# kangxiongbin/HyLight

Measured on AMD Instinct MI355X. Metric: long-read all-vs-all overlaps/sec, higher is better.
Workload: dtype u8/int32

## Files before the change

hylight_amd/csrc/ava_align.hip:

```cpp
#include <algorithm>
#include <memory>
#include <type_traits>

#include "ava_internal.h"
#include "dev_prims.h"
#include "wave_ops.h"

namespace hlmi {

namespace {
constexpr int WG = 256;
constexpr int WAVES = WG / 64;
constexpr int SEQ_T_MAX = EXT_MAX + BAND_W;
constexpr int NR_SHORT = 128;
constexpr int WIDE_SHORT = 128;
inline dim3 grid1(size_t n) { return grid_for(n, WG); }

struct Task {
    uint32_t piece;
    uint16_t kind;
    uint16_t narrow;
    uint64_t qa, ta;
    int16_t m, n;
    int16_t dlo;
    int16_t trim;
};
constexpr uint16_t TASK_REV = 4;
constexpr uint16_t TASK_ONE = 8;
struct TaskOut {
    int32_t score;
    int32_t bi, bj;
    uint32_t runs_off, n_runs;
    uint32_t pad;
};
__device__ __forceinline__ uint32_t end_codes(uint32_t first_run, uint32_t last_run) { return (first_run & 15u) | (last_run & 15u) << 4; }

__global__ void piece_task_count_kernel(const Piece *pieces, size_t n, uint32_t *cnt) {
    size_t i = blockIdx.x * (size_t)blockDim.x + threadIdx.x;
    if (i < n) cnt[i] = pieces[i].n_fp + 1;
}

struct TaskRef { uint32_t pk, fp; };
struct PieceGeom {
    uint64_t qo, to;
    uint32_t ql, tl;
    uint32_t strand;
    uint32_t stub_cand;
};
struct TaskGeom {
    const TaskRef *ref;
    const PieceGeom *pg;
    const FixPt *fps;
};
__device__ __forceinline__ Task build_task(const PieceGeom &p, uint32_t piece, uint32_t kind, FixPt f0, FixPt f1, int ext_max) {
    const int ql = (int)p.ql, tl = (int)p.tl;
    const uint64_t qo = p.qo, to = p.to;
    const uint16_t rev = p.strand ? TASK_REV : 0;
    auto qaddr = [&](int pos) { return p.strand ? qo + (uint64_t)(ql - 1 - pos) : qo + (uint64_t)pos; };
    if (kind == 1) {
        const int qs = (int)f0.q, ts = (int)f0.t;
        const int m = qs < ext_max ? qs : ext_max, n2 = ts < m + BAND_W ? ts : m + BAND_W;
        return Task{piece, (uint16_t)(1u | rev), (uint16_t)(qs <= ext_max ? (qs + 1) << 1 : 0), qaddr(qs - 1),
                    to + (uint64_t)(ts - 1), (int16_t)m, (int16_t)n2, (int16_t)(-(BAND_W / 2 - 1)), 0};
    }
    if (kind == 2) {
        const int qe = (int)f0.q, te = (int)f0.t;
        const int m = ql - qe < ext_max ? ql - qe : ext_max, n2 = tl - te < m + BAND_W ? tl - te : m + BAND_W;
        return Task{piece, (uint16_t)(2u | rev), (uint16_t)(ql - qe <= ext_max ? (ql - qe + 1) << 1 : 0), qaddr(qe),
// ... 51 lines not shown
    if (stub_oh >= 0) {
        const FixPt a = fps[p.fp_off], b = fps[p.fp_off + p.n_fp - 1];
        const uint32_t dq = (uint32_t)(ext_max + stub_oh), dt = (uint32_t)(ext_max + BAND_W + stub_oh);
        cand = ((a.q > dq && a.t > dt) || (ql - b.q > dq && tl - b.t > dt)) ? 1u : 0u;
    }
    pg[i] = PieceGeom{qoff[p.q], toff[p.t], ql, tl, p.strand, cand};
}

struct AlignArgs {
    Task *tasks;
    TaskGeom geom;
    size_t n_tasks;
    const uint32_t *list;
    size_t n_list;
    const uint8_t *qcodes, *tcodes;
    long long q_total, t_total;
    const uint8_t *qpacked, *tpacked;
    const uint32_t *qnflag, *tnflag;
    int match, mismatch, go, ge, ambi;
    int go2, ge2;
    int end_bonus;
    int ext_max;
    int ext_all_long;
    int ungapped;
    int kmax;
    int kgap1;
    int kgap2;
    int one_ok;
    int kext_plain;
    int kext_bonus;
    int trim_ok;
    int kshift;
    TaskOut *out;
    uint32_t *runs;
    uint32_t cap_runs;
    uint32_t *counters;
    uint32_t run_buf_cap;
    uint8_t *cls_bare;
    uint8_t *defer_flag;
    const uint32_t *defer_list, *defer_count;
};

__device__ __forceinline__ uint32_t wave_excl_sum_u32(uint32_t v, int lane, uint32_t &total) {
    (void)lane;
    const uint32_t x = wave_prefix_sum_incl_dpp(v);
    total = (uint32_t)__builtin_amdgcn_readlane((int)x, 63);
    return x - v;
}

constexpr uint32_t RUN_CHUNK = 4096;
constexpr uint32_t RUN_CHUNK_SMALL = 256;
__device__ __forceinline__ uint32_t pool_take(const AlignArgs &a, uint32_t n, uint32_t &chunk_off, uint32_t &chunk_left,
                                              bool &ok, uint32_t chunk = RUN_CHUNK) {
    if (n > chunk_left) {
        const uint32_t want = n > chunk ? n : chunk;
        chunk_off = atomicAdd(&a.counters[0], want);
        chunk_left = want;
        if ((unsigned long long)chunk_off + want > a.cap_runs) { a.counters[1] = 1; chunk_left = 0; ok = false; return 0; }
    }
    const uint32_t off = chunk_off;
    chunk_off += n;
    chunk_left -= n;
    return off;
}

__device__ __forceinline__ uint32_t load_codes4(const uint8_t *base, long long idx, long long total) {
    if (idx >= 0 && idx + 4 <= total) {
        uint32_t v;
        __builtin_memcpy(&v, base + idx, 4);
        return v;
    }
    uint32_t v = 0;
    for (int k = 0; k < 4; ++k) v |= (uint32_t)(idx + k >= 0 && idx + k < total ? base[idx + k] : 4) << (8 * k);
    return v;
}
__device__ __forceinline__ uint32_t comp_codes4(uint32_t x) {
    const uint32_t n = x & 0x04040404u;
    return (x ^ 0x03030303u) & ~((n >> 1) | (n >> 2));
}
__device__ __forceinline__ uint32_t load_window4(const uint8_t *codes, long long total, long long a0, bool down, bool comp, int x) {
    uint32_t v = down ? __builtin_bswap32(load_codes4(codes, a0 - x - 3, total)) : load_codes4(codes, a0 + x, total);
    if (comp) v = comp_codes4(v);
    return v;
}

__device__ __forceinline__ uint32_t load_window4p(const uint8_t *codes, long long a0, bool down, bool comp, int x) {
    uint32_t v;
    __builtin_memcpy(&v, codes + (down ? a0 - x - 3 : a0 + x), 4);
    if (down) v = __builtin_bswap32(v);
    if (comp) v = comp_codes4(v);
    return v;
}


enum { ST_BASES = 0, ST_BASES_SQUARE, ST_BASES_NARROW, ST_BASES_WIDE, ST_FAST, ST_DP, ST_DP_ROWS, ST_NARROW_SMALL, ST_WIDE_ONE, ST_STUB_EXT, ST_EXT_CERT, ST_EXT_DP_ROW, ST_EXT_DP_K, ST_LONG, ST_BASES_LONG, ST_PACKED, N_ALIGN_STATS };
constexpr int NR_SMALL = 64;
constexpr uint8_t CLS_LONG = 5;
constexpr uint8_t CLS_LONG32 = 7;
constexpr uint8_t CLS_UNGAPPED = 6;

__device__ __forceinline__ uint64_t load_codes8(const uint8_t *base, long long idx, long long total) {
    if (idx >= 0 && idx + 8 <= total) {
        uint64_t v;
        __builtin_memcpy(&v, base + idx, 8);
        return v;
    }
    uint64_t v = 0;
    for (int k = 0; k < 8; ++k) v |= (uint64_t)(idx + k >= 0 && idx + k < total ? base[idx + k] : 4) << (8 * k);
    return v;
}
__device__ __forceinline__ uint64_t load_window8(const uint8_t *codes, long long total, long long a0, bool down, bool comp, int x) {
    uint64_t v = down ? __builtin_bswap64(load_codes8(codes, a0 - x - 7, total)) : load_codes8(codes, a0 + x, total);
    if (comp) {
        const uint64_t n = v & 0x0404040404040404ull;
        v = (v ^ 0x0303030303030303ull) & ~((n >> 1) | (n >> 2));
    }
    return v;
}

__device__ __forceinline__ uint64_t load_window8p(const uint8_t *codes, long long a0, bool down, bool comp, int x) {
    uint64_t v;
    __builtin_memcpy(&v, codes + (down ? a0 - x - 7 : a0 + x), 8);
    if (down) v = __builtin_bswap64(v);
    if (comp) {
        const uint64_t n = v & 0x0404040404040404ull;
        v = (v ^ 0x0303030303030303ull) & ~((n >> 1) | (n >> 2));
    }
    return v;
// ... 37 lines not shown
    for (uint32_t w = g0 >> 5; w <= g1 >> 5; ++w) {
        uint32_t keep = ~0u;
        if (w == g0 >> 5) keep &= ~0u << (g0 & 31);
        if (w == g1 >> 5) keep &= ~0u >> (31 - (g1 & 31));
        any |= nflag[w] & keep;
    }
    return any != 0;
}
__device__ __forceinline__ bool window_flagged(const uint32_t *nflag, long long a0, bool down, int len) {
    return down ? range_flagged(nflag, a0 - (len - 1), a0) : range_flagged(nflag, a0, a0 + (len - 1));
}

template <int PASS>
__global__ __launch_bounds__(WG) __attribute__((amdgpu_waves_per_eu(PASS == 1 ? 4 : 5))) void classify_kernel(AlignArgs a, uint8_t *cls, unsigned long long *stats) {
    __shared__ unsigned long long s_stat[WAVES][N_ALIGN_STATS];
    constexpr int CMP_WORDS = PASS == 1 ? 64 * (BLOCK_MAX / 32) : 1;
    __shared__ uint32_t s_mm[WAVES][CMP_WORDS], s_up[WAVES][CMP_WORDS], s_dn[WAVES][CMP_WORDS];
    __shared__ uint64_t s_qa[WAVES][PASS == 1 ? 64 : 1], s_ta[WAVES][PASS == 1 ? 64 : 1];
    __shared__ uint32_t s_geo[WAVES][PASS == 1 ? 64 : 1], s_amb[WAVES][2];
    const int lane = threadIdx.x & 63;
    const size_t tid = blockIdx.x * (size_t)blockDim.x + threadIdx.x;
    const size_t n_thr = (size_t)gridDim.x * blockDim.x;
    uint32_t chunk_off = 0, chunk_left = 0;
    uint32_t st[N_ALIGN_STATS] = {};
    const size_t n_units = PASS == 1 ? a.n_tasks : (size_t)*a.defer_count;
    const size_t rounds = (n_units + n_thr - 1) / n_thr;
    TaskRef ref_n{0, 0};
    uint32_t ti_n = 0;
    if (PASS == 1) { if (tid < n_units) ref_n = a.geom.ref[tid]; }
    else if (tid < n_units) ti_n = a.defer_list[tid];
    for (size_t r = 0; r < rounds; ++r) {
        const size_t u = r * n_thr + tid;
        bool live = u < n_units;
        const size_t ti = PASS == 1 || !live ? u : (size_t)ti_n;
        TaskRef ref = ref_n;
        if (PASS == 2 && live) ref = a.geom.ref[ti];
        {
            const size_t un = u + n_thr;
            if (PASS == 1) { if (un < n_units) ref_n = a.geom.ref[un]; }
            else if (un < n_units) ti_n = a.defer_list[un];
        }
        Task tk{};
        bool held = false;
        bool bare = false;
        if (live) {
            const uint32_t pc = ref.pk & 0x3fffffffu, kind = ref.pk >> 30;
            const PieceGeom pg = a.geom.pg[pc];
            held = PASS == 1 && kind != 0 && pg.stub_cand != 0;
            bare = a.cls_bare != nullptr && pg.stub_cand != 0;
            const FixPt f0 = a.geom.fps[ref.fp];
            FixPt f1{0, 0};
            if (kind == 0) f1 = a.geom.fps[ref.fp + 1];
            tk = build_task(pg, pc, kind, f0, f1, a.ext_max);
        }
        const int m = tk.m, n = tk.n;
        uint8_t c = 2;
        bool try_fast = false;
        if (live) {
            if (m <= 0 || n <= 0 || held) c = 0;
            else if ((tk.kind & 3) == 0) {
                if (m > BLOCK_MAX || n > BLOCK_MAX)
                    c = (n > m ? n - m : m - n) <= HALF_DELTA ? CLS_LONG32 : CLS_LONG;
                else { c = tk.narrow ? (m <= NR_SHORT ? 1 : 3) : 2; try_fast = (m == n); }
            } else if ((m < n - tk.dlo ? m : n - tk.dlo) > EXT_MAX) { c = CLS_LONG32; tk.dlo = (int16_t)(-(HALF_W / 2 - 1)); }
            else if (a.ext_all_long) c = CLS_LONG;
            if (c == 2 && (m < n - tk.dlo ? m : n - tk.dlo) <= WIDE_SHORT) c = 4;
// ... 318 lines not shown
                        const int xp = k ? xpos2 : xpos;
                        if (xp < from || xp >= to) continue;
                        if (xp > prev) runs[nr++] = (uint32_t)(xp - prev) << 4 | OP_EQ;
                        if (nr && xp == prev && prev > from && (runs[nr - 1] & 15u) == OP_X) runs[nr - 1] += 1u << 4;
                        else runs[nr++] = 1u << 4 | OP_X;
                        prev = xp + 1;
                    }
                    if (to > prev) runs[nr++] = (uint32_t)(to - prev) << 4 | OP_EQ;
                };
                seg(0, p_star);
                runs[nr++] = (uint32_t)gap << 4 | (del ? OP_D : OP_I);
                seg(p_star, mn);
                const int subs = (xpos >= 0 ? 1 : 0) + (xpos2 >= 0 ? 1 : 0);
                int gap_cost = a.go + a.ge * gap;
                if (a.go2 && a.go2 + a.ge2 * gap < gap_cost) gap_cost = a.go2 + a.ge2 * gap;
                fast_score = a.match * (mn - subs) - a.mismatch * subs - gap_cost;
                fast = true;
                c = 0;
            }
        } else if (fast) {
            c = 0;
            int prev = 0, xs = -1, xe = -1;
            for (int i = 0; i < k; ++i) {
                const int x = mpos[i];
                if (x == xe) { xe = x + 1; continue; }
                if (xs >= 0) { runs[nr++] = (uint32_t)(xe - xs) << 4 | OP_X; prev = xe; }
                if (x > prev) runs[nr++] = (uint32_t)(x - prev) << 4 | OP_EQ;
                xs = x; xe = x + 1;
            }
            if (xs >= 0) { runs[nr++] = (uint32_t)(xe - xs) << 4 | OP_X; prev = xe; }
            if (m > prev) runs[nr++] = (uint32_t)(m - prev) << 4 | OP_EQ;
        }
        if (bare) nr = 0;
        uint32_t wave_total;
        const uint32_t mine = wave_excl_sum_u32(nr, lane, wave_total);
        uint32_t base = 0;
        bool ok = true;
        if (wave_total) {
            if (lane == 0) base = pool_take(a, wave_total, chunk_off, chunk_left, ok);
            base = (uint32_t)__shfl((int)base, 0, 64);
            ok = __shfl((int)ok, 0, 64) != 0;
        }
        if (fast) {
            if (ok) for (uint32_t q = 0; q < nr; ++q) a.runs[base + mine + q] = runs[q];
            const bool ext = (tk.kind & 3) != 0;
            const int L = ext_take >= 0 ? ext_take : (m < n ? m : n);
            a.out[ti] = TaskOut{fast_score, ext ? L : m, ext ? L : n, base + mine, ok ? nr : 0, (nr ? end_codes(runs[0], runs[nr - 1]) : 0u) | ext_flag};
        } else if (live && c == 0) {
            a.out[ti] = TaskOut{0, 0, 0, 0, 0, 0};
        }
        int m_dp = m;
        if (live && !fast && (c == 1 || c == 3) && a.kmax >= 0 && last_x >= 0 && a.trim_ok && !a.ungapped) {
            const int mn = m < n ? m : n;
            int T = mn - 1 - last_x;
            T = T < mn - 1 ? T : mn - 1;
            if (T > 0) {
                tk.m = (int16_t)(m - T); tk.n = (int16_t)(n - T); tk.trim = (int16_t)T;
                m_dp = m - T;
                c = m_dp <= NR_SHORT ? 1 : 3;
            }
        }
        if (live) {
            if (a.ungapped && c != 0) c = CLS_UNGAPPED;
            cls[ti] = bare ? 0 : c;
            if (a.cls_bare) a.cls_bare[ti] = bare ? c : 0;
            if (c != 0) a.tasks[ti] = tk;
            if (held) ++st[ST_STUB_EXT];
            else if (m > 0 && n > 0) {
                const uint32_t bases = (uint32_t)(m + n);
                st[ST_BASES] += bases;
                if ((tk.kind & 3) == 0 && m == n) st[ST_BASES_SQUARE] += bases;
                if (c == 0) ++st[ST_FAST];
                else {
                    ++st[ST_DP];
                    if (c == CLS_LONG || c == CLS_LONG32) { ++st[ST_LONG]; st[ST_BASES_LONG] += bases; st[ST_DP_ROWS] += (uint32_t)(m < n - tk.dlo ? m : n - tk.dlo); }
                    else if (c == 2 || c == 4) { st[ST_BASES_WIDE] += bases; st[ST_DP_ROWS] += (uint32_t)(m < n - tk.dlo ? m : n - tk.dlo); }
                    else { st[ST_BASES_NARROW] += bases; st[ST_DP_ROWS] += (uint32_t)m_dp; if (c == 1 && m_dp < NR_SMALL && !bare) ++st[ST_NARROW_SMALL]; }
                }
            }
        }
    }
// ... 1249 lines not shown
            base = (uint32_t)__shfl((int)base, 0, 64);
            ok = __shfl((int)ok, 0, 64) != 0;
        }
        if (live && ok && n_runs) {
            uint32_t k = 0, len = 0;
            int op_cur = -1;
            uint32_t *dst = a.runs + base + mine;
            auto put = [&]() { dst[left ? n_runs - 1 - k : k] = len << 4 | (uint32_t)op_cur; ++k; };
            for (int x = 0; x < take; x += 8) {
                uint64_t q8, t8;
                pair_at(x, q8, t8);
                const int lim = take - x < 8 ? take - x : 8;
                for (int y = 0; y < lim; ++y) {
                    const int op = ((q8 >> (8 * y)) & 0xff) == ((t8 >> (8 * y)) & 0xff) ? (int)OP_EQ : (int)OP_X;
                    if (op != op_cur) { if (len) put(); op_cur = op; len = 0; }
                    ++len;
                }
            }
            if (len) put();
        }
        if (live) {
            const uint32_t ends = n_runs ? (left ? end_codes(last_op, first_op) : end_codes(first_op, last_op)) : 0u;
            a.out[ti] = TaskOut{out_score, ext ? take : (int)tk.m, ext ? take : (int)tk.n, base + mine, ok ? n_runs : 0,
                                ends | (ext && take == end_row ? 0x80000000u : 0u)};
        }
    }
}

struct AsmArgs {
    const Piece *pieces;
    const FixPt *fps;
    const uint32_t *task_off;
    const TaskOut *tout;
    const uint32_t *runs;
    size_t n_pieces;
    const uint32_t *qlen, *tlen, *rank_q, *rank_t, *chunk_of_t;
    int min_dp_score, end_bonus;
    const uint32_t *plist;
    const PieceGeom *pg;
    uint8_t *late;
    int stub_score;
    int bare;
    uint32_t stage_cap;
};

constexpr uint32_t ASM_MID = 4;
constexpr int ASM_STAGE = 1024;
template <bool WRITE>
__global__ __launch_bounds__(WG) void assemble_kernel(AsmArgs a, uint32_t *n_ops, uint8_t *valid, const uint64_t *ops_off,
                                                       uint32_t *ops, PafRec *recs, uint64_t *ord_hi, uint64_t *ord_lo) {
    __shared__ uint32_t s_stage[WRITE ? WAVES : 1][WRITE ? ASM_STAGE : 1];
    uint32_t *const stage = s_stage[WRITE ? (threadIdx.x >> 6) : 0];
    const int lane = threadIdx.x & 63;
    const size_t wave = (blockIdx.x * (size_t)blockDim.x + threadIdx.x) >> 6;
    const size_t n_waves = ((size_t)gridDim.x * blockDim.x) >> 6;
    for (size_t idx = wave; idx < a.n_pieces; idx += n_waves) {
        const size_t i = !WRITE && a.plist ? (size_t)a.plist[idx] : idx;
        if (WRITE && !valid[i]) continue;
        const Piece p = a.pieces[i];
        const FixPt *fp = a.fps + p.fp_off;
        const TaskOut *to = a.tout + a.task_off[i];
        const uint32_t n_tasks = p.n_fp + 1;
        const bool bare = a.bare && a.pg[i].stub_cand != 0;
        uint32_t *w = WRITE ? ops + ops_off[i] : nullptr;
        long long score = 0;
        unsigned long long nmatch = 0, blen = 0;
        uint32_t slots = 0;
        uint32_t carry_code = 99;
        constexpr uint32_t NO_SLOT = 0xffffffffu;
        uint32_t open_idx = NO_SLOT, open_val = 0;
        int ext_l_i = 0, ext_l_j = 0, ext_r_i = 0, ext_r_j = 0;
        TaskOut r_next{0, 0, 0, 0, 0, 0};
        if ((uint32_t)lane < n_tasks) r_next = to[lane];
        for (uint32_t t0 = 0; t0 < n_tasks; t0 += 64) {
            const uint32_t t = t0 + (uint32_t)lane;
            TaskOut r = r_next;
            r_next = TaskOut{0, 0, 0, 0, 0, 0};
            if (t + 64 < n_tasks) r_next = to[t + 64];
            bool keep = false;
            if (t < n_tasks) {
                keep = true;
                if (t == 0 || t == n_tasks - 1)
                    keep = !(r.score + ((r.pad & 0x80000000u) ? a.end_bonus : 0) <= 0 || (r.n_runs == 0 && !bare));
            }
            if (keep && t == 0) { ext_l_i = r.bi; ext_l_j = r.bj; }
            if (keep && t == n_tasks - 1 && t != 0) { ext_r_i = r.bi; ext_r_j = r.bj; }
            long long sc = keep ? r.score : 0;
            const uint32_t nr = keep && !bare ? r.n_runs : 0;
            const uint32_t first = r.pad & 15u, last = (r.pad >> 4) & 15u;
            const unsigned long long ne_mask = __ballot(nr != 0);
            const unsigned long long below = ne_mask & ((1ull << lane) - 1ull);
            const int prev_lane = below ? 63 - __clzll((long long)below) : 0;
            const uint32_t prev_last = (uint32_t)__shfl((int)last, prev_lane, 64);
            const uint32_t prev_code = below ? (prev_last & 15u) : carry_code;
            const bool mrg = nr != 0 && (first & 15u) == prev_code;
            uint32_t tot_runs, tot_mrg;
            const uint32_t S = wave_excl_sum_u32(nr, lane, tot_runs);
            const uint32_t Mx = wave_excl_sum_u32(mrg ? 1u : 0u, lane, tot_mrg);
            if (WRITE) {
                const uint32_t F = nr ? a.runs[r.runs_off] : 0u;
                const uint32_t L = nr >= 2 ? a.runs[r.runs_off + nr - 1] : F;
                uint32_t mid[ASM_MID];
#pragma unroll
                for (uint32_t u = 0; u < ASM_MID; ++u) mid[u] = u + 3 <= nr ? a.runs[r.runs_off + 1 + u] : 0u;
                const uint32_t P = wave_prefix_sum_incl_dpp(mrg ? F >> 4 : 0u);
                const bool opens = nr != 0 && (!mrg || nr >= 2);
                const unsigned long long om = __ballot(opens);
                const uint32_t P_end = (uint32_t)__builtin_amdgcn_readlane((int)P, 63);
                const uint32_t T0 = om ? (uint32_t)__shfl((int)P, __ffsll((long long)om) - 1, 64) : P_end;
                open_val += T0 << 4;
                if (om && open_idx != NO_SLOT && lane == 0) w[open_idx] = open_val;
                const unsigned long long above = lane == 63 ? 0ull : om & ~((2ull << lane) - 1ull);
                const uint32_t P_next = (uint32_t)__shfl((int)P, above ? __ffsll((long long)above) - 1 : 63, 64);
                const uint32_t base = slots + S - (Mx + (mrg ? 1u : 0u));
                const uint32_t own_slot = base + (nr ? nr - 1 : 0u);
                const uint32_t own_val = L + ((P_next - P) << 4);
                const uint32_t n_out = tot_runs - tot_mrg;
                const bool staged = n_out <= a.stage_cap;
                auto put = [&](uint32_t slot, uint32_t v) { if (staged) stage[slot - slots] = v; else w[slot] = v; };
                if (om) {
                    const int lb = 63 - __clzll((long long)om);
                    open_idx = (uint32_t)__builtin_amdgcn_readlane((int)own_slot, lb);
                    open_val = (uint32_t)__builtin_amdgcn_readlane((int)own_val, lb);
                    if (opens && lane != lb) put(own_slot, own_val);
                }
                if (nr) {
                    blen += F >> 4;
                    if ((F & 15u) == OP_EQ) nmatch += F >> 4;
                }
                if (nr >= 2) {
                    blen += L >> 4;
                    if ((L & 15u) == OP_EQ) nmatch += L >> 4;
                    if (!mrg) put(base, F);
// ... 42 lines not shown
        for (int o = 32; o > 0; o >>= 1) { nmatch += __shfl_xor(nmatch, o, 64); blen += __shfl_xor(blen, o, 64); }
        if (lane == 0) {
            if (open_idx != NO_SLOT) w[open_idx] = open_val;
            const int qs = (int)fp[0].q - li, ts = (int)fp[0].t - lj;
            const int qe = (int)fp[p.n_fp - 1].q + ri, te = (int)fp[p.n_fp - 1].t + rj;
            const uint32_t ql = a.qlen[p.q];
            PafRec r{};
            r.qid = a.rank_q[p.q]; r.tid = a.rank_t[p.t];
            r.qlen = ql; r.tlen = a.tlen[p.t];
            r.qs = p.strand ? ql - (uint32_t)qe : (uint32_t)qs;
            r.qe = p.strand ? ql - (uint32_t)qs : (uint32_t)qe;
            r.ts = (uint32_t)ts; r.te = (uint32_t)te;
            r.nmatch = (uint32_t)nmatch; r.blen = (uint32_t)blen;
            r.flags = p.strand ? PF_REV : 0;
            r.chunk = a.chunk_of_t[p.t];
            r.cig_off = ops_off[i]; r.cig_n = slots; r.tie = 0;
            recs[i] = r;
            ord_hi[i] = (uint64_t)r.chunk << 32 | p.q;
            ord_lo[i] = (uint64_t)p.t << 43 | (uint64_t)p.strand << 42 | (uint64_t)(p.chain & 0x3fffffu) << 20 | (p.piece & 0xfffffu);
        }
    }
}

template <bool WRITE>
__global__ __launch_bounds__(WG) void assemble_lane_kernel(AsmArgs a, uint32_t *n_ops, uint8_t *valid, const uint64_t *ops_off,
                                                            uint32_t *ops, PafRec *recs, uint64_t *ord_hi, uint64_t *ord_lo) {
    const size_t idx = blockIdx.x * (size_t)blockDim.x + threadIdx.x;
    if (idx >= a.n_pieces) return;
    const size_t i = !WRITE && a.plist ? (size_t)a.plist[idx] : idx;
    if (WRITE && !valid[i]) return;
    const Piece p = a.pieces[i];
    const FixPt *fp = a.fps + p.fp_off;
    const TaskOut *to = a.tout + a.task_off[i];
    const uint32_t n_tasks = p.n_fp + 1;
    const bool bare = a.bare && a.pg[i].stub_cand != 0;
    uint32_t *w = WRITE ? ops + ops_off[i] : nullptr;
    long long score = 0;
    unsigned long long nmatch = 0, blen = 0;
    uint32_t slots = 0;
    uint32_t pend = 0;
    uint32_t carry_code = 99;
    int li = 0, lj = 0, ri = 0, rj = 0;
    for (uint32_t t = 0; t < n_tasks; ++t) {
        const TaskOut r = to[t];
        bool keep = true;
        if (t == 0 || t == n_tasks - 1)
            keep = !(r.score + ((r.pad & 0x80000000u) ? a.end_bonus : 0) <= 0 || (r.n_runs == 0 && !bare));
        if (!keep) continue;
        if (t == 0) { li = r.bi; lj = r.bj; }
        else if (t == n_tasks - 1) { ri = r.bi; rj = r.bj; }
        score += r.score;
        const uint32_t nr = bare ? 0u : r.n_runs;
        if (!nr) continue;
        const uint32_t first = r.pad & 15u, last = (r.pad >> 4) & 15u;
        const bool mrg = first == carry_code;
        carry_code = last;
        if (!WRITE) {
            slots += nr - (mrg ? 1u : 0u);
            continue;
        }
        for (uint32_t x = 0; x < nr; ++x) {
            const uint32_t run = a.runs[r.runs_off + x];
            blen += run >> 4;
            if ((run & 15u) == OP_EQ) nmatch += run >> 4;
            if (x == 0 && mrg) pend += (run >> 4) << 4;
            else {
                if (pend) w[slots++] = pend;
                pend = run;
            }
        }
    }
    if (!WRITE) {
        const bool ok = (slots > 0 || bare) && score >= a.min_dp_score;
        valid[i] = ok ? 1 : 0;
        n_ops[i] = ok ? slots : 0;
        if (a.late) a.late[i] = a.pg[i].stub_cand && !((slots > 0 || bare) && score >= a.stub_score) ? 1 : 0;
        return;
    }
    if (pend) w[slots++] = pend;
    const int qs = (int)fp[0].q - li, ts = (int)fp[0].t - lj;
    const int qe = (int)fp[p.n_fp - 1].q + ri, te = (int)fp[p.n_fp - 1].t + rj;
    const uint32_t ql = a.qlen[p.q];
    PafRec r{};
    r.qid = a.rank_q[p.q]; r.tid = a.rank_t[p.t];
    r.qlen = ql; r.tlen = a.tlen[p.t];
    r.qs = p.strand ? ql - (uint32_t)qe : (uint32_t)qs;
    r.qe = p.strand ? ql - (uint32_t)qs : (uint32_t)qe;
    r.ts = (uint32_t)ts; r.te = (uint32_t)te;
    r.nmatch = (uint32_t)nmatch; r.blen = (uint32_t)blen;
    r.flags = p.strand ? PF_REV : 0;
    r.chunk = a.chunk_of_t[p.t];
    r.cig_off = ops_off[i]; r.cig_n = slots; r.tie = 0;
    recs[i] = r;
    ord_hi[i] = (uint64_t)r.chunk << 32 | p.q;
    ord_lo[i] = (uint64_t)p.t << 43 | (uint64_t)p.strand << 42 | (uint64_t)(p.chain & 0x3fffffu) << 20 | (p.piece & 0xfffffu);
// ... 112 lines not shown
    const size_t wave = (blockIdx.x * (size_t)blockDim.x + threadIdx.x) >> 6;
    const size_t n_waves = ((size_t)gridDim.x * blockDim.x) >> 6;
    for (size_t i = wave; i < n; i += n_waves) {
        const Piece p = pieces[i];
        const uint32_t to = off[i];
        for (uint32_t k = (uint32_t)lane; k < p.n_fp; k += 64) dst[to + k] = src[p.fp_off + k];
        if (lane == 0) pieces[i].fp_off = fp_base + to;
    }
}
}

struct PieceSpan { struct { const Piece *p; } pieces; size_t n_pieces, n_fp; struct { const FixPt *p; } fps; };
static void align_span(const AvaInput &in, const hlmi_ava_opts &o, const uint32_t *d_qlen, const uint32_t *d_tlen,
                       const PieceSpan &ch, AlignOut &out) {
    out = AlignOut();
    const size_t P = ch.n_pieces;
    if (!P) return;
    DBuf<uint32_t> tcnt(P), toff(P);
    hipLaunchKernelGGL(piece_task_count_kernel, grid1(P), dim3(WG), 0, stream(), ch.pieces.p, P, tcnt.p);
    exclusive_scan_u32(tcnt.p, toff.p, P);
    const size_t NT = ch.n_fp + P;
    DBuf<Task> tasks(NT);
    if (P >= (1u << 30)) fail(HLMI_EINVAL, "more than 2^30 alignment pieces in one batch");
    DBuf<TaskRef> task_ref(NT);
    DBuf<PieceGeom> pgeom(P);
    if (NT <= 17 * P)
        hipLaunchKernelGGL(task_ref_lane_kernel, grid1(P), dim3(WG), 0, stream(), ch.pieces.p, toff.p, P, d_qlen, d_tlen, in.Q->off.p, in.T->off.p,
                           ch.fps.p, o.stub_oh, ext_rows(o), task_ref.p, pgeom.p);
    else
    hipLaunchKernelGGL(task_ref_kernel, dim3((unsigned)std::min<size_t>(cdiv(P, (size_t)WAVES), 256 * 32)), dim3(WG), 0, stream(),
                       ch.pieces.p, toff.p, P, d_qlen, d_tlen, in.Q->off.p, in.T->off.p, ch.fps.p, o.stub_oh, ext_rows(o), task_ref.p, pgeom.p);
    HIP_CHECK(hipGetLastError());
    DBuf<TaskOut> tout(NT);
    DBuf<uint32_t> counters(2);
    DBuf<unsigned long long> astats(N_ALIGN_STATS);
    constexpr size_t MAX_BLOCKS = 256 * 16;
    const size_t open_chunks = MAX_BLOCKS * (4 * WAVES * RUN_CHUNK + 2 * 4 * WAVES * RUN_CHUNK_SMALL) +
                               (size_t)3 * 256 * 32 * 8 * PK_WAVES * RUN_CHUNK_SMALL;
    size_t run_share = std::max<size_t>(NT * 12, 1 << 16);
    DBuf<uint32_t> runs;
    AsmArgs as{};
    as.pieces = ch.pieces.p; as.fps = ch.fps.p; as.task_off = toff.p; as.tout = tout.p; as.n_pieces = P;
    as.min_dp_score = o.min_dp_score; as.end_bonus = o.end_bonus;
    as.qlen = d_qlen; as.tlen = d_tlen; as.rank_q = in.d_rank_q; as.rank_t = in.d_rank_t; as.chunk_of_t = in.d_chunk_of_t;
    as.pg = pgeom.p; as.stub_score = o.min_dp_score + std::max(0, o.end_bonus);
    as.stage_cap = (uint32_t)ASM_STAGE;
    if (const char *e = hook("HLMI_ASM_STAGE_CAP")) as.stage_cap = (uint32_t)std::min(ASM_STAGE, std::max(0, atoi(e)));
    DBuf<uint32_t> nops(P);
    DBuf<uint8_t> valid(P), late(o.stub_oh >= 0 ? P : 0);
    DBuf<uint32_t> late_idx(o.stub_oh >= 0 ? P : 0);
    size_t n_late = 0;
    const unsigned nba = (unsigned)std::min<size_t>(cdiv(P, (size_t)WAVES), 256 * 32);
    const bool small_pieces = NT <= 17 * P && !hook("HLMI_ASM_WAVE");
    const int worst = std::max(std::max(o.match, o.mismatch), std::max(o.ambi, o.gap_open + o.gap_ext));
    const bool packed = worst > 0 && (long long)worst * (BLOCK_MAX + NARROW_W + 2) <= 4000 && o.match >= 0 && o.mismatch >= 0 &&
                        o.ambi >= 0 && o.gap_open >= 0 && o.gap_ext >= 0 && !hook("HLMI_NARROW_UNPACKED");
    const bool bare = o.stub_oh >= 0 && packed && !hook("HLMI_STUB_FULL_ROWS");
    as.bare = bare ? 1 : 0;
    if (long_rows_cap(o) > 32000) fail(HLMI_EINVAL, "max_gap %d: alignment tasks are limited to 32 000 rows", o.max_gap);
    bool ext_all_long = false;
    if (o.zdrop > 0) {
        const int D = std::max(std::max(o.mismatch, o.ambi), o.gap_open + o.gap_ext);
        const int rows_down = D > 0 ? (o.zdrop + D - 1) / D : EXT_MAX;
        ext_all_long = (long long)o.match * (EXT_MAX - rows_down) + std::max(o.end_bonus, 0) > o.zdrop;
    }
    const uint32_t long_chunks_cap = (uint32_t)(long_rows_cap(o) + 31) / 32, long_runs_cap = (uint32_t)(2 * long_rows_cap(o) + 64);
    constexpr unsigned LONG_BLOCKS_MAX = 256 * 8;
    struct LongLaunch { DBuf<uint32_t> list, planes, runs, ctl; };
    std::vector<std::unique_ptr<LongLaunch>> long_launches;
    struct LongReady { AlignArgs al; LongArgs la; unsigned nb; bool half, tb; const char *timer; };
    std::vector<LongReady> long_ready;
    hipEvent_t long_done = nullptr;
    bool long_pending = false, long_on_side = false;
    struct SideGuard {
        ~SideGuard() { if (hipStream_t s = side_stream_if_created()) (void)hipStreamSynchronize(s); }
// ... 49 lines not shown
        aa.ext_max = ext_rows(o);
        aa.ext_all_long = ext_all_long ? 1 : 0;
        aa.ungapped = o.bandwidth == 0 ? 1 : 0;
        aa.match = o.match; aa.mismatch = o.mismatch; aa.go = o.gap_open; aa.ge = o.gap_ext; aa.ambi = o.ambi;
        aa.go2 = o.gap_open2 > 0 ? o.gap_open2 : 0; aa.ge2 = o.gap_open2 > 0 ? o.gap_ext2 : 0;
        if (aa.go2 && aa.go2 + aa.ge2 * (NARROW_W - 1) < aa.go + aa.ge * (NARROW_W - 1))
            fail(HLMI_EINVAL, "two-piece gap cost: the second piece must not be the cheaper one below %d bases", NARROW_W);
        {
            const int den = o.match + o.mismatch, num = o.match + 2 * (o.gap_open + o.gap_ext);
            aa.kmax = den > 0 && num > 0 ? std::min(3, (num - 1) / den) : 0;
            if (o.match <= 0 || o.gap_open < 0 || o.gap_ext <= 0) aa.kmax = -1;
            const int k = aa.kmax + 1, U = den, T = num;
            aa.kgap1 = aa.kmax >= 0 && U < o.gap_open + 2 * o.gap_ext + o.match && !hook("HLMI_NO_GAP1_CERT") ? 1 : 0;
            {
                auto c = [&](int L) { int v = o.gap_open + o.gap_ext * L; if (o.gap_open2 > 0) v = std::min(v, o.gap_open2 + o.gap_ext2 * L); return v; };
                aa.kgap2 = aa.kgap1 && U < o.match + c(2) && 2 * U < o.match + 2 * c(1) && 2 * U < 2 * o.match + c(2) + c(3) - c(1) &&
                           c(2) == o.gap_open + 2 * o.gap_ext && c(1) == o.gap_open + o.gap_ext && !hook("HLMI_NO_GAP2_CERT") ? 1 : 0;
            }
            aa.kshift = aa.kmax >= 0 && k <= 3 && k * U > T && k * U < T + o.match + std::min(2 * o.gap_ext, o.gap_open + o.gap_ext) &&
                        !hook("HLMI_NO_SHIFT_CERT") ? 1 : 0;
        }
        aa.trim_ok = hook("HLMI_NO_SUFFIX_TRIM") ? 0 : 1;
        aa.one_ok = hook("HLMI_NO_ONE_PIECE_CERT") ? 0 : 1;
        {
            const int U = o.match + o.mismatch;
            int G = o.gap_open + o.gap_ext;
            if (aa.go2 > 0) G = std::min(G, aa.go2 + aa.ge2);
            const bool sane = aa.kmax >= 0 && o.match > 0 && o.mismatch >= 0 && !hook("HLMI_NO_EXT_CERT");
            aa.kext_plain = sane && G >= U && U < 2 * G + o.match ? 1 : 0;
            aa.kext_bonus = 0;
            for (int k = 1; k <= 2; ++k)
                if (sane && o.end_bonus > 0 && k * U < G && k * U < o.end_bonus + o.match && k * U < 2 * G + o.match) aa.kext_bonus = k;
        }
        aa.out = tout.p; aa.runs = runs.p; aa.cap_runs = (uint32_t)cap_runs; aa.counters = counters.p;
        as.runs = runs.p;
        aa.run_buf_cap = 0xffffffffu;
        if (const char *e = hook("HLMI_RUN_BUF_CAP")) aa.run_buf_cap = (uint32_t)std::max(0, atoi(e));
        DBuf<uint8_t> cls(NT), f1(NT), cls_bare(bare ? NT : 0);
        DBuf<uint32_t> list1(NT), list2(NT), list3(NT), list4(NT);
        DBuf<uint32_t> list_n(4);
        aa.cls_bare = bare ? cls_bare.p : nullptr;
        auto class_list = [&](const uint8_t *cls_arr, uint8_t v) -> size_t {
            if (long_flag.n < NT) { long_flag.alloc(NT); long_list.alloc(NT); }
            hipLaunchKernelGGL(class_flag_kernel, grid1(NT), dim3(WG), 0, stream(), cls_arr, NT, v, long_flag.p);
            select_flagged_indices_async(long_flag.p, long_list.p, NT, long_n.p);
            return (size_t)long_n.download(1)[0];
        };
        auto run_ungapped = [&](const uint8_t *cls_arr, bool tb) -> size_t {
            if (!aa.ungapped) return 0;
            const size_t nl = class_list(cls_arr, CLS_UNGAPPED);
            if (!nl) return 0;
            aa.list = long_list.p; aa.n_list = nl;
            note_list("align_ungapped", tasks.p, long_list.p, nl);
            KTimer kt("align_ungapped");
            const unsigned nb = (unsigned)std::min<size_t>(cdiv(nl, (size_t)WG), MAX_BLOCKS);
            if (tb) hipLaunchKernelGGL(align_ungapped_kernel<true>, dim3(nb), dim3(WG), 0, stream(), aa, o.zdrop);
            else hipLaunchKernelGGL(align_ungapped_kernel<false>, dim3(nb), dim3(WG), 0, stream(), aa, o.zdrop);
            HIP_CHECK(hipGetLastError());
            return nl;
        };
        auto run_long_class = [&](const uint8_t *cls_arr, bool tb, uint8_t cv) -> size_t {
            const bool half = cv == CLS_LONG32;
            const char *timer = half ? (tb ? "align_long32" : "align_score_long32") : (tb ? "align_long" : "align_score_long");
            const size_t nl = class_list(cls_arr, cv);
            if (!nl) return 0;
            note_list(timer, tasks.p, long_list.p, nl);
            hipLaunchKernelGGL(list_ext_kernel, dim3((unsigned)std::min<size_t>(cdiv(nl, (size_t)WG), 1024)), dim3(WG), 0, stream(), tasks.p,
// ... 237 lines not shown
                }
                as.plist = late_idx.p; as.n_pieces = n_late;
                const unsigned nbl = (unsigned)std::min<size_t>(cdiv(n_late, (size_t)WAVES), 256 * 32);
                join_long();
                {
                    KTimer kt("assemble_count");
                    if (small_pieces) hipLaunchKernelGGL(assemble_lane_kernel<false>, grid1(as.n_pieces), dim3(WG), 0, stream(), as, nops.p, valid.p,
                                                         nullptr, nullptr, nullptr, nullptr, nullptr);
                    else
                    hipLaunchKernelGGL(assemble_kernel<false>, dim3(nbl), dim3(WG), 0, stream(), as, nops.p, valid.p, nullptr, nullptr,
                                       nullptr, nullptr, nullptr);
                }
                as.plist = nullptr; as.n_pieces = P;
            }
        }
        if (attempt == 0) {
            stat_add("align_tasks_narrow", (double)(n1 + n3)); stat_add("align_tasks_wide", (double)(n2 + n4 + (bare ? 0 : n_wide_late)));
            stat_add("align_tasks_score_only", (double)n_bare_tasks);
            stat_add("align_tasks_long", (double)n_long_tb); stat_add("align_tasks_long_score_only", (double)n_long_bare);
        }
        HIP_CHECK(hipGetLastError());
        join_long();
        std::vector<uint32_t> hc = counters.download(2);
        check_long();
        if (!hc[1]) break;
        if (attempt >= 3) fail(HLMI_ENOMEM, "CIGAR run pool overflow");
        run_share *= 4;
    }
    stat_add("align_tasks", (double)NT);
    {
        std::vector<unsigned long long> h = astats.download(N_ALIGN_STATS);
        stat_add("align_tasks_fast", (double)h[ST_FAST]);
        stat_add("align_tasks_packed", (double)h[ST_PACKED]);
        stat_add("align_tasks_dp", (double)h[ST_DP]);
        stat_add("align_dp_rows", (double)h[ST_DP_ROWS]);
        stat_add("align_dp_bases", (double)h[ST_BASES]);
        stat_add("align_bases_classify", (double)h[ST_BASES_SQUARE]);
        stat_add("align_bases_narrow", (double)h[ST_BASES_NARROW]);
        stat_add("align_bases_wide", (double)h[ST_BASES_WIDE]);
        stat_add("align_bases_long", (double)h[ST_BASES_LONG]);
        const std::vector<unsigned long long> lb = lb_bases.download(N_LB + 2);
        stat_add("align_long_rows_run", long_rows_run);
        stat_add("align_long_ext", (double)lb[N_LB]);
        stat_add("align_long_ext_rows", (double)lb[N_LB + 1]);
        for (int k = 0; k < N_LB; ++k)
            if (lb_n[k] > 0) {
                stat_add(std::string("align_n.") + LB_NAMES[k], lb_n[k]);
                stat_add(std::string("align_bases.") + LB_NAMES[k], (double)lb[k]);
            }
        stat_add("align_tasks_wide_one_piece", (double)h[ST_WIDE_ONE]);
        stat_add("align_ext_certified", (double)h[ST_EXT_CERT]);
        stat_add("align_ext_dp_bonus_row_elsewhere", (double)h[ST_EXT_DP_ROW]);
        stat_add("align_ext_dp_substitutions", (double)h[ST_EXT_DP_K]);
        stat_add("align_ext_held", (double)h[ST_STUB_EXT]);
        stat_add("align_ext_late", (double)(2 * n_late));
    }
    if (o.stub_oh < 0) {
        KTimer kt("assemble_count");
        if (small_pieces) hipLaunchKernelGGL(assemble_lane_kernel<false>, grid1(as.n_pieces), dim3(WG), 0, stream(), as, nops.p, valid.p,
                                             nullptr, nullptr, nullptr, nullptr, nullptr);
        else
        hipLaunchKernelGGL(assemble_kernel<false>, dim3(nba), dim3(WG), 0, stream(), as, nops.p, valid.p, nullptr, nullptr,
                           nullptr, nullptr, nullptr);
    }
    HIP_CHECK(hipGetLastError());
    DBuf<uint64_t> ooff(P);
// ... 113 lines not shown
```

hylight_amd/csrc/runtime.cpp:

```cpp
#include <mutex>

#include "common.h"
#include <sched.h>

#include <iterator>

namespace hlmi {

namespace {
thread_local std::string g_last_error;
bool g_ready = false;
int g_device = 0;
int g_threads = 0;
std::map<std::string, double> g_stats;
std::mutex g_mu;
std::mutex g_stat_mu;

struct KRec { std::string name; hipEvent_t a, b; hipStream_t s; };
struct Lane {
    hipStream_t stream = nullptr, side = nullptr;
    std::vector<KRec> krecs;
    void *pinned = nullptr;
};
Lane g_lanes[MAX_LANES];
// ... 140 lines not shown
    "HLMI_ANCHOR_BATCH_M",
    "HLMI_ANCHOR_PAIRS",
    "HLMI_ANCHOR_SPLIT",
    "HLMI_ASM_STAGE_CAP",
    "HLMI_ASM_WAVE",
    "HLMI_CHAIN_DP16_CHECK",
    "HLMI_CHAIN_NO_DP16",
    "HLMI_CHAIN_NO_SMALL",
    "HLMI_SEED_GROUP", "HLMI_TEXT_GPU", "HLMI_TEXT_HOST", "HLMI_GRAPH_WINDOW_MB", "HLMI_LANES", "HLMI_SET_ASIDE_CUTS", "HLMI_SEED_NO_GUESS",
    "HLMI_CHAIN_PROF",
    "HLMI_CHAIN_UNPACKED",
    "HLMI_CLASSIFY_BYTES",
    "HLMI_GROUP_HIST",
    "HLMI_HOST_TIMERS",
    "HLMI_LONG_SIDE_STREAM",
    "HLMI_NARROW_LONG_UNPACKED",
    "HLMI_NARROW_UNPACKED",
    "HLMI_NO_EXT_CERT",
    "HLMI_POLISH_ROWS_GRID",
    "HLMI_NO_GAP1_CERT",
    "HLMI_NO_GAP2_CERT",
    "HLMI_NO_ONE_PIECE_CERT",
    "HLMI_NO_RANK_WORD",
    "HLMI_NO_SHIFT_CERT",
    "HLMI_NO_STUB",
    "HLMI_NO_SUFFIX_TRIM",
    "HLMI_QCAP_MIN",
    "HLMI_RUN_BUF_CAP",
    "HLMI_SKETCH_PART_MBASES",
    "HLMI_SNP_SORT",
    "HLMI_STUB_FULL_ROWS",
    "HLMI_SUBRUN_MAX_MANCHORS",
    "HLMI_SUBRUN_MAX_OUT_MB",
    "HLMI_SUBRUN_MBASES"};
std::unordered_map<std::string, std::string> g_hooks;
}
void hooks_refresh() {
    g_hooks.clear();
    for (const char *n : HOOK_NAMES)
        if (const char *v = getenv(n)) g_hooks[n] = v;
}
const char *hook(const char *name) {
    bool known = false;
    for (const char *n : HOOK_NAMES) known = known || strcmp(n, name) == 0;
    if (!known) fail(HLMI_EINVAL, "hook %s is not in the table of runtime.cpp", name);
    auto it = g_hooks.find(name);
    return it == g_hooks.end() ? nullptr : it->second.c_str();
}

namespace {
struct CachedBlock { void *p; int lane; };
std::multimap<size_t, CachedBlock> g_free_blocks;
std::mutex g_pool_mu;
std::unordered_map<void *, size_t> g_block_size;
size_t g_pooled_bytes = 0;
size_t g_owned_bytes = 0;
size_t g_peak_in_use = 0;
constexpr size_t POOL_CAP = 160ull << 30;
constexpr size_t GRAN = 2ull << 20;
}

static size_t size_class(size_t bytes) {
    size_t want = (bytes + GRAN - 1) / GRAN * GRAN;
    if (want > (64ull << 20)) {
        size_t p2 = 1;
        while ((p2 << 1) <= want) p2 <<= 1;
        const size_t step = p2 >> 3;
// ... 132 lines not shown
```

Before: 3684.

## Encode exact-match fast tasks as compact result words instead of TaskOut and runs

After: 3670. No clear change (-0.4%).

```diff
diff --git a/hylight_amd/csrc/ava_align.hip b/hylight_amd/csrc/ava_align.hip
--- a/hylight_amd/csrc/ava_align.hip
+++ b/hylight_amd/csrc/ava_align.hip
@@ -34,6 +34,19 @@
     uint32_t pad;
 };
 __device__ __forceinline__ uint32_t end_codes(uint32_t first_run, uint32_t last_run) { return (first_run & 15u) | (last_run & 15u) << 4; }
+
+constexpr uint32_t RES_COMPACT = 0x80000000u;
+__device__ __forceinline__ uint32_t compact_run(uint32_t word) { return (word & ~RES_COMPACT) << 4 | OP_EQ; }
+__device__ __forceinline__ TaskOut compact_out(uint32_t word, int match) {
+    const int m = (int)(word & ~RES_COMPACT);
+    return TaskOut{match * m, m, m, 0, 1, end_codes(OP_EQ, OP_EQ)};
+}
+__device__ __forceinline__ TaskOut task_result(uint32_t word, const TaskOut *to, uint32_t t, int match) {
+    return (word & RES_COMPACT) ? compact_out(word, match) : to[t];
+}
+__device__ __forceinline__ TaskOut task_result(uint32_t word, const TaskOut &rec, int match) {
+    return (word & RES_COMPACT) ? compact_out(word, match) : rec;
+}
 
 __global__ void piece_task_count_kernel(const Piece *pieces, size_t n, uint32_t *cnt) {
     size_t i = blockIdx.x * (size_t)blockDim.x + threadIdx.x;
@@ -151,6 +164,8 @@
     int trim_ok;
     int kshift;
     TaskOut *out;
+    uint32_t *res;
+    int compact_ok;
     uint32_t *runs;
     uint32_t cap_runs;
     uint32_t *counters;
@@ -212,7 +227,7 @@
 }
 
 
-enum { ST_BASES = 0, ST_BASES_SQUARE, ST_BASES_NARROW, ST_BASES_WIDE, ST_FAST, ST_DP, ST_DP_ROWS, ST_NARROW_SMALL, ST_WIDE_ONE, ST_STUB_EXT, ST_EXT_CERT, ST_EXT_DP_ROW, ST_EXT_DP_K, ST_LONG, ST_BASES_LONG, ST_PACKED, N_ALIGN_STATS };
+enum { ST_BASES = 0, ST_BASES_SQUARE, ST_BASES_NARROW, ST_BASES_WIDE, ST_FAST, ST_DP, ST_DP_ROWS, ST_NARROW_SMALL, ST_WIDE_ONE, ST_STUB_EXT, ST_EXT_CERT, ST_EXT_DP_ROW, ST_EXT_DP_K, ST_LONG, ST_BASES_LONG, ST_PACKED, ST_COMPACT, N_ALIGN_STATS };
 constexpr int NR_SMALL = 64;
 constexpr uint8_t CLS_LONG = 5;
 constexpr uint8_t CLS_LONG32 = 7;
@@ -316,6 +331,7 @@
     for (size_t r = 0; r < rounds; ++r) {
         const size_t u = r * n_thr + tid;
         bool live = u < n_units;
+        const bool in_range = live;
         const size_t ti = PASS == 1 || !live ? u : (size_t)ti_n;
         TaskRef ref = ref_n;
         if (PASS == 2 && live) ref = a.geom.ref[ti];
@@ -700,6 +716,9 @@
             if (m > prev) runs[nr++] = (uint32_t)(m - prev) << 4 | OP_EQ;
         }
         if (bare) nr = 0;
+        const bool compact = PASS == 1 && fast && a.compact_ok && (tk.kind & 3) == 0 && m == n && k == 0 && !bare && !held;
+        if (compact) { nr = 0; ++st[ST_COMPACT]; }
+        if (PASS == 1 && in_range) a.res[ti] = compact ? RES_COMPACT | (uint32_t)m : 0u;
         uint32_t wave_total;
         const uint32_t mine = wave_excl_sum_u32(nr, lane, wave_total);
         uint32_t base = 0;
@@ -709,12 +728,12 @@
             base = (uint32_t)__shfl((int)base, 0, 64);
             ok = __shfl((int)ok, 0, 64) != 0;
         }
-        if (fast) {
+        if (fast && !compact) {
             if (ok) for (uint32_t q = 0; q < nr; ++q) a.runs[base + mine + q] = runs[q];
             const bool ext = (tk.kind & 3) != 0;
             const int L = ext_take >= 0 ? ext_take : (m < n ? m : n);
             a.out[ti] = TaskOut{fast_score, ext ? L : m, ext ? L : n, base + mine, ok ? nr : 0, (nr ? end_codes(runs[0], runs[nr - 1]) : 0u) | ext_flag};
-        } else if (live && c == 0) {
+        } else if (live && c == 0 && !compact) {
             a.out[ti] = TaskOut{0, 0, 0, 0, 0, 0};
         }
         int m_dp = m;
@@ -2030,6 +2049,8 @@
     const FixPt *fps;
     const uint32_t *task_off;
     const TaskOut *tout;
+    const uint32_t *res;
+    int match;
     const uint32_t *runs;
     size_t n_pieces;
     const uint32_t *qlen, *tlen, *rank_q, *rank_t, *chunk_of_t;
@@ -2045,7 +2066,7 @@
 constexpr uint32_t ASM_MID = 4;
 constexpr int ASM_STAGE = 1024;
 template <bool WRITE>
-__global__ __launch_bounds__(WG) void assemble_kernel(AsmArgs a, uint32_t *n_ops, uint8_t *valid, const uint64_t *ops_off,
+__global__ __launch_bounds__(WG) __attribute__((amdgpu_waves_per_eu(WRITE ? 6 : 8))) void assemble_kernel(AsmArgs a, uint32_t *n_ops, uint8_t *valid, const uint64_t *ops_off,
                                                        uint32_t *ops, PafRec *recs, uint64_t *ord_hi, uint64_t *ord_lo) {
     __shared__ uint32_t s_stage[WRITE ? WAVES : 1][WRITE ? ASM_STAGE : 1];
     uint32_t *const stage = s_stage[WRITE ? (threadIdx.x >> 6) : 0];
@@ -2058,6 +2079,7 @@
         const Piece p = a.pieces[i];
         const FixPt *fp = a.fps + p.fp_off;
         const TaskOut *to = a.tout + a.task_off[i];
+        const uint32_t *rs = a.res + a.task_off[i];
         const uint32_t n_tasks = p.n_fp + 1;
         const bool bare = a.bare && a.pg[i].stub_cand != 0;
         uint32_t *w = WRITE ? ops + ops_off[i] : nullptr;
@@ -2068,13 +2090,20 @@
         constexpr uint32_t NO_SLOT = 0xffffffffu;
         uint32_t open_idx = NO_SLOT, open_val = 0;
         int ext_l_i = 0, ext_l_j = 0, ext_r_i = 0, ext_r_j = 0;
+        uint32_t word_next = 0, word_next2 = 0;
         TaskOut r_next{0, 0, 0, 0, 0, 0};
-        if ((uint32_t)lane < n_tasks) r_next = to[lane];
+        if ((uint32_t)lane < n_tasks) { word_next = rs[lane]; r_next = to[lane]; }
+        if ((uint32_t)lane + 64 < n_tasks) word_next2 = rs[lane + 64];
+        r_next = task_result(word_next, r_next, a.match);
         for (uint32_t t0 = 0; t0 < n_tasks; t0 += 64) {
             const uint32_t t = t0 + (uint32_t)lane;
+            const uint32_t word = word_next;
             TaskOut r = r_next;
+            word_next = word_next2;
+            word_next2 = 0;
+            if (t + 128 < n_tasks) word_next2 = rs[t + 128];
             r_next = TaskOut{0, 0, 0, 0, 0, 0};
-            if (t + 64 < n_tasks) r_next = to[t + 64];
+            if (t + 64 < n_tasks) r_next = task_result(word_next, to, t + 64, a.match);
             bool keep = false;
             if (t < n_tasks) {
                 keep = true;
@@ -2096,7 +2125,7 @@
             const uint32_t S = wave_excl_sum_u32(nr, lane, tot_runs);
             const uint32_t Mx = wave_excl_sum_u32(mrg ? 1u : 0u, lane, tot_mrg);
             if (WRITE) {
-                const uint32_t F = nr ? a.runs[r.runs_off] : 0u;
+                const uint32_t F = nr ? ((word & RES_COMPACT) ? compact_run(word) : a.runs[r.runs_off]) : 0u;
                 const uint32_t L = nr >= 2 ? a.runs[r.runs_off + nr - 1] : F;
                 uint32_t mid[ASM_MID];
 #pragma unroll
@@ -2205,6 +2234,7 @@
     const Piece p = a.pieces[i];
     const FixPt *fp = a.fps + p.fp_off;
     const TaskOut *to = a.tout + a.task_off[i];
+    const uint32_t *rs = a.res + a.task_off[i];
     const uint32_t n_tasks = p.n_fp + 1;
     const bool bare = a.bare && a.pg[i].stub_cand != 0;
     uint32_t *w = WRITE ? ops + ops_off[i] : nullptr;
@@ -2215,7 +2245,8 @@
     uint32_t carry_code = 99;
     int li = 0, lj = 0, ri = 0, rj = 0;
     for (uint32_t t = 0; t < n_tasks; ++t) {
-        const TaskOut r = to[t];
+        const uint32_t word = rs[t];
+        const TaskOut r = task_result(word, to[t], a.match);
         bool keep = true;
         if (t == 0 || t == n_tasks - 1)
             keep = !(r.score + ((r.pad & 0x80000000u) ? a.end_bonus : 0) <= 0 || (r.n_runs == 0 && !bare));
@@ -2233,7 +2264,7 @@
             continue;
         }
         for (uint32_t x = 0; x < nr; ++x) {
-            const uint32_t run = a.runs[r.runs_off + x];
+            const uint32_t run = (word & RES_COMPACT) ? compact_run(word) : a.runs[r.runs_off + x];
             blen += run >> 4;
             if ((run & 15u) == OP_EQ) nmatch += run >> 4;
             if (x == 0 && mrg) pend += (run >> 4) << 4;
@@ -2412,6 +2443,7 @@
                        ch.pieces.p, toff.p, P, d_qlen, d_tlen, in.Q->off.p, in.T->off.p, ch.fps.p, o.stub_oh, ext_rows(o), task_ref.p, pgeom.p);
     HIP_CHECK(hipGetLastError());
     DBuf<TaskOut> tout(NT);
+    DBuf<uint32_t> res(NT);
     DBuf<uint32_t> counters(2);
     DBuf<unsigned long long> astats(N_ALIGN_STATS);
     constexpr size_t MAX_BLOCKS = 256 * 16;
@@ -2420,7 +2452,7 @@
     size_t run_share = std::max<size_t>(NT * 12, 1 << 16);
     DBuf<uint32_t> runs;
     AsmArgs as{};
-    as.pieces = ch.pieces.p; as.fps = ch.fps.p; as.task_off = toff.p; as.tout = tout.p; as.n_pieces = P;
+    as.pieces = ch.pieces.p; as.fps = ch.fps.p; as.task_off = toff.p; as.tout = tout.p; as.res = res.p; as.match = o.match; as.n_pieces = P;
     as.min_dp_score = o.min_dp_score; as.end_bonus = o.end_bonus;
     as.qlen = d_qlen; as.tlen = d_tlen; as.rank_q = in.d_rank_q; as.rank_t = in.d_rank_t; as.chunk_of_t = in.d_chunk_of_t;
     as.pg = pgeom.p; as.stub_score = o.min_dp_score + std::max(0, o.end_bonus);
@@ -2536,7 +2568,8 @@
             for (int k = 1; k <= 2; ++k)
                 if (sane && o.end_bonus > 0 && k * U < G && k * U < o.end_bonus + o.match && k * U < 2 * G + o.match) aa.kext_bonus = k;
         }
-        aa.out = tout.p; aa.runs = runs.p; aa.cap_runs = (uint32_t)cap_runs; aa.counters = counters.p;
+        aa.out = tout.p; aa.res = res.p; aa.compact_ok = hook("HLMI_TASK_COMPACT_OFF") ? 0 : 1;
+        aa.runs = runs.p; aa.cap_runs = (uint32_t)cap_runs; aa.counters = counters.p;
         as.runs = runs.p;
         aa.run_buf_cap = 0xffffffffu;
         if (const char *e = hook("HLMI_RUN_BUF_CAP")) aa.run_buf_cap = (uint32_t)std::max(0, atoi(e));
@@ -2840,6 +2873,7 @@
         std::vector<unsigned long long> h = astats.download(N_ALIGN_STATS);
         stat_add("align_tasks_fast", (double)h[ST_FAST]);
         stat_add("align_tasks_packed", (double)h[ST_PACKED]);
+        stat_add("align_tasks_compact", (double)h[ST_COMPACT]);
         stat_add("align_tasks_dp", (double)h[ST_DP]);
         stat_add("align_dp_rows", (double)h[ST_DP_ROWS]);
         stat_add("align_dp_bases", (double)h[ST_BASES]);
diff --git a/hylight_amd/csrc/runtime.cpp b/hylight_amd/csrc/runtime.cpp
--- a/hylight_amd/csrc/runtime.cpp
+++ b/hylight_amd/csrc/runtime.cpp
@@ -196,7 +196,8 @@
     "HLMI_STUB_FULL_ROWS",
     "HLMI_SUBRUN_MAX_MANCHORS",
     "HLMI_SUBRUN_MAX_OUT_MB",
-    "HLMI_SUBRUN_MBASES"};
+    "HLMI_SUBRUN_MBASES",
+    "HLMI_TASK_COMPACT_OFF"};
 std::unordered_map<std::string, std::string> g_hooks;
 }
 void hooks_refresh() {
```
